# tuannv-github/srsRAN_Project

Measured on AMD Instinct MI355X. Metric: PDSCH+PUSCH codeblocks/s @ 100 MHz 273-PRB 4x4 MIMO (PDSCH 4 layers, PUSCH 4 layers x 4 rx), higher is better.
Workload: dtype int8+fp32; 1 GPU; BASELINE metric (PDSCH+PUSCH codeblocks/s @ 100 MHz 273-PRB 4x4 MIMO): full PDSCH+PUSCH slot pipeline, 100 MHz numerology-1 273 PRB, 256QAM R=948/1024; parallelism=single GPU

## Files before the change

srsran_project_amd/csrc/crc_api.cpp:

```cpp
#include "srsran_amd/crc.h"

#include <hip/hip_runtime.h>

#include "api_common.h"
#include "crc_args.h"
#include "crc_internal.h"
#include "ldpc_common.h"
#include <mutex>
#include <vector>

using namespace srs_amd;

struct srs_amd_crc_calculator {
  int         device   = 0;
  int         poly     = 0;
  uint32_t    polynom  = 0;
  int         order    = 0;
  uint32_t    max_bits = 0;
  uint32_t*   d_table  = nullptr;
  hipStream_t stream   = nullptr;
  void*       scratch  = nullptr;
  size_t      scratch_size = 0;
  uint32_t*   d_acc        = nullptr;
  uint32_t    acc_rows     = 0;
  std::mutex  mtx;
  ~srs_amd_crc_calculator()
  {
    (void)hipSetDevice(device);
    if (stream) {
      (void)hipStreamSynchronize(stream);
      (void)hipStreamDestroy(stream);
    }
    (void)hipFree(d_table);
    (void)hipFree(scratch);
    (void)hipFree(d_acc);
  }
};

namespace {

int check_rows(srs_amd_crc_calculator* crc, uint32_t stride, uint32_t nof_bits, uint32_t extra)
{
  if (crc == nullptr) {
    return fail(SRS_AMD_EINVAL, "null CRC calculator");
  }
  if (nof_bits > crc->max_bits) {
    return fail(SRS_AMD_EINVAL, "message of %u bits exceeds the calculator's %u", nof_bits, crc->max_bits);
  }
  if (static_cast<uint64_t>(stride) * 8 < static_cast<uint64_t>(nof_bits) + extra) {
    return fail(SRS_AMD_EINVAL, "row stride %u bytes too small for %u bits", stride, nof_bits + extra);
  }
  return SRS_AMD_OK;
}

int launch(srs_amd_crc_calculator* crc, uint32_t* d_out, uint8_t* d_bits, uint32_t stride, uint32_t nof_bits,
           uint32_t nof_rows, bool attach, hipStream_t stream)
{
  crc_args a{};
  a.bits      = d_bits;
  a.checksums = d_out;
  a.table     = crc->d_table;
  a.stride    = stride;
  a.nof_bits  = nof_bits;
  a.polynom   = crc->polynom;
  a.order     = static_cast<uint32_t>(crc->order);
  a.attach    = attach ? 1 : 0;
  hipError_t e = hipSetDevice(crc->device);
  if (e == hipSuccess && crc_needs_accumulator(nof_bits)) {
    if (crc->acc_rows < nof_rows) {
      (void)hipFree(crc->d_acc);
      crc->d_acc    = nullptr;
      crc->acc_rows = 0;
      e             = hipMalloc(&crc->d_acc, sizeof(uint32_t) * nof_rows);
      if (e == hipSuccess) {
        crc->acc_rows = nof_rows;
      }
    }
    a.acc = crc->d_acc;
  }
  if (e == hipSuccess) {
    e = launch_crc(a, nof_rows, stream);
  }
  return e == hipSuccess ? SRS_AMD_OK : hip_fail(e, "crc_kernel launch");
}

}

extern "C" {

int srs_amd_crc_calculator_create(srs_amd_crc_calculator** out, int poly, uint32_t max_bits, int device)
{
  if (out == nullptr) {
    return fail(SRS_AMD_EINVAL, "null handle pointer");
  }
  *out             = nullptr;
  uint32_t polynom = 0;
  int      order   = 0;
  if (!crc_params(poly, polynom, order)) {
    return fail(SRS_AMD_EINVAL, "Invalid CRC polynomial %d.", poly);
  }
  if (max_bits == 0 || max_bits > (1u << 26)) {
    return fail(SRS_AMD_EINVAL, "max_bits %u out of range", max_bits);
  }
  int rc = select_device(device);
  if (rc != SRS_AMD_OK) {
    return rc;
  }
  auto* c     = new srs_amd_crc_calculator();
  c->device   = device;
  c->poly     = poly;
  c->polynom  = polynom;
  c->order    = order;
  c->max_bits = max_bits;
  std::vector<uint32_t> t = crc_linear_table(poly, static_cast<int>(max_bits) + 32);
  hipError_t            e = hipMalloc(&c->d_table, t.size() * sizeof(uint32_t));
  if (e == hipSuccess) {
    e = hipMemcpy(c->d_table, t.data(), t.size() * sizeof(uint32_t), hipMemcpyHostToDevice);
  }
  if (e == hipSuccess) {
    e = hipStreamCreateWithFlags(&c->stream, hipStreamNonBlocking);
  }
  if (e != hipSuccess) {
    delete c;
    return hip_fail(e, "CRC table");
  }
  *out = c;
  return SRS_AMD_OK;
}

void srs_amd_crc_calculator_destroy(srs_amd_crc_calculator* crc)
{
  delete crc;
}

uint32_t srs_amd_crc_order(const srs_amd_crc_calculator* crc)
{
  return crc ? static_cast<uint32_t>(crc->order) : 0;
}

int srs_amd_crc_calculate_batch(srs_amd_crc_calculator* crc,
                                uint32_t*               d_checksums,
                                const uint8_t*          d_bits,
                                uint32_t                stride,
                                uint32_t                nof_bits,
                                uint32_t                nof_rows,
                                void*                   stream)
{
  int rc = check_rows(crc, stride, nof_bits, 0);
  if (rc != SRS_AMD_OK) {
    return rc;
  }
  if (nof_rows == 0) {
    return SRS_AMD_OK;
  }
  if (d_checksums == nullptr || (d_bits == nullptr && nof_bits > 0)) {
    return fail(SRS_AMD_EINVAL, "null device buffer");
  }
  std::lock_guard<std::mutex> lock(crc->mtx);
  return launch(crc, d_checksums, const_cast<uint8_t*>(d_bits), stride, nof_bits, nof_rows, false,
                static_cast<hipStream_t>(stream));
}

int srs_amd_crc_attach_batch(srs_amd_crc_calculator* crc,
                             uint8_t*                d_bits,
                             uint32_t                stride,
                             uint32_t                nof_bits,
                             uint32_t                nof_rows,
                             void*                   stream)
{
  int rc = check_rows(crc, stride, nof_bits, crc ? static_cast<uint32_t>(crc->order) : 0);
  if (rc != SRS_AMD_OK) {
// ... 10 lines not shown
}

int srs_amd_crc_calculate(srs_amd_crc_calculator* crc, uint32_t* checksum, const uint8_t* bits, uint32_t nof_bits)
{
  const uint32_t nbytes = (nof_bits + 7) / 8;
  int            rc     = check_rows(crc, nbytes, nof_bits, 0);
  if (rc != SRS_AMD_OK) {
    return rc;
  }
  if (checksum == nullptr || (bits == nullptr && nof_bits > 0)) {
    return fail(SRS_AMD_EINVAL, "null argument");
  }
  std::lock_guard<std::mutex> lock(crc->mtx);
  hipError_t                  e = hipSetDevice(crc->device);
  const size_t                need = 64 + nbytes;
  if (e == hipSuccess && need > crc->scratch_size) {
    (void)hipFree(crc->scratch);
    crc->scratch      = nullptr;
    crc->scratch_size = 0;
    e                 = hipMalloc(&crc->scratch, need);
    if (e == hipSuccess) {
      crc->scratch_size = need;
    }
  }
  if (e != hipSuccess) {
    return hip_fail(e, "CRC scratch");
  }
  auto* d_crc  = static_cast<uint32_t*>(crc->scratch);
  auto* d_bits = static_cast<uint8_t*>(crc->scratch) + 64;
  if (nbytes > 0) {
    e = hipMemcpyAsync(d_bits, bits, nbytes, hipMemcpyHostToDevice, crc->stream);
  }
  if (e != hipSuccess) {
    return hip_fail(e, "CRC upload");
  }
  rc = launch(crc, d_crc, d_bits, nbytes, nof_bits, 1, false, crc->stream);
  if (rc != SRS_AMD_OK) {
    return rc;
  }
  e = hipMemcpyAsync(checksum, d_crc, sizeof(uint32_t), hipMemcpyDeviceToHost, crc->stream);
  if (e == hipSuccess) {
    e = hipStreamSynchronize(crc->stream);
  }
  return e == hipSuccess ? SRS_AMD_OK : hip_fail(e, "CRC download");
}

}

const uint32_t* srs_amd::crc_device_table(const srs_amd_crc_calculator* crc)
{
  return crc ? crc->d_table : nullptr;
}

uint32_t srs_amd::crc_polynom(const srs_amd_crc_calculator* crc)
{
  return crc ? crc->polynom : 0;
}

uint32_t srs_amd::crc_order(const srs_amd_crc_calculator* crc)
{
  return crc ? static_cast<uint32_t>(crc->order) : 0;
}
```

srsran_project_amd/csrc/crc_device.h:

```cpp
#pragma once

#include <hip/hip_runtime.h>

#include <cstdint>

namespace srs_amd {

__device__ __forceinline__ uint32_t crc_wave_xor(uint32_t v)
{
#pragma unroll
  for (int o = 32; o >= 1; o >>= 1) {
    v ^= static_cast<uint32_t>(__shfl_xor(static_cast<int>(v), o, 64));
  }
  return v;
}

template <int THREADS>
__device__ __forceinline__ void crc_table8_init(uint32_t* T, uint32_t order, uint32_t polynom)
{
  if (order < 8) {
    return;
  }
  const uint32_t highbit = 1u << order;
  for (uint32_t t = threadIdx.x; t < 256; t += THREADS) {
// ... 73 lines not shown

__device__ __forceinline__ uint32_t crc_move(uint32_t R, uint32_t d, uint32_t order, const uint32_t* table)
{
  uint32_t out = 0;
#pragma unroll
  for (uint32_t j = 0; j < CRC_MAX_ORDER; ++j) {
    const uint32_t k    = j + d;
    const uint32_t word = k >= order ? table[k - order] : 0u;
    const uint32_t v    = k < order ? (1u << (k & 31u)) : word;
    out ^= (j < order) ? (v & (0u - ((R >> j) & 1u))) : 0u;
  }
  return out;
}

template <typename Fetch>
__device__ __forceinline__ uint32_t crc_chunk_rem(const Fetch& fetch, uint32_t b0, uint32_t b1, uint32_t order,
                                                  const uint32_t* T)
{
  const uint32_t mask = (1u << order) - 1u;
  const uint32_t sh   = order - 8;
  uint32_t       r    = 0;
  for (uint32_t b = b0; b < b1; b += CRC_FETCH_BATCH) {
    uint32_t v[CRC_FETCH_BATCH];
#pragma unroll
    for (uint32_t k = 0; k < CRC_FETCH_BATCH; ++k) {
      v[k] = b + k < b1 ? fetch(b + k) : 0u;
    }
#pragma unroll
    for (uint32_t k = 0; k < CRC_FETCH_BATCH; ++k) {
      if (b + k < b1) {
        r = T[r >> sh] ^ ((r << 8) & mask) ^ v[k];
      }
    }
  }
  return r;
}

__device__ __forceinline__ uint32_t crc_mulmod(uint32_t a, uint32_t c, uint32_t order, uint32_t polynom)
{
  const uint32_t mask = (1u << order) - 1u;
  const uint32_t top  = 1u << (order - 1);
  uint32_t       r    = 0;
#pragma unroll
  for (uint32_t i = 0; i < CRC_MAX_ORDER; ++i) {
    if (i < order) {
      r ^= c & (0u - ((a >> i) & 1u));
      const uint32_t hi = c & top;
      c                 = ((c << 1) & mask) ^ (hi ? (polynom & mask) : 0u);
    }
  }
  return r;
}

__device__ __forceinline__ uint32_t crc_xpow(uint32_t m, uint32_t order, const uint32_t* table)
{
  return m < order ? (1u << m) : table[m - order];
}

template <int THREADS>
__device__ __forceinline__ uint32_t crc_block_xor(uint32_t v, uint32_t* partial)
{
  v = crc_wave_xor(v);
  __syncthreads();
  if ((threadIdx.x & 63) == 0) {
    partial[threadIdx.x >> 6] = v;
  }
  __syncthreads();
  uint32_t crc = 0;
#pragma unroll
  for (int w = 0; w < THREADS / 64; ++w) {
    crc ^= partial[w];
  }
  return crc;
}

template <int THREADS, typename Fetch>
__device__ uint32_t block_crc_bytes(const Fetch&    fetch,
                                    uint32_t        n,
                                    uint32_t        order,
                                    uint32_t        polynom,
                                    const uint32_t* table,
                                    const uint32_t* T,
                                    uint32_t*       partial)
{
  const uint32_t nbytes = (n + 7) / 8;
  const uint32_t per    = (nbytes + THREADS - 1) / THREADS;
  const uint32_t b0     = threadIdx.x * per;
  const uint32_t b1     = min(nbytes, b0 + per);
  return crc_block_xor<THREADS>(crc_chunk_contrib(fetch, b0, b1, n, order, polynom, table, T), partial);
}

__device__ __forceinline__ void attach_crc_bits(uint8_t* row, uint32_t n, uint32_t order, uint32_t crc)
{
  const uint32_t first = n >> 3, last = (n + order - 1) >> 3;
  uint32_t       bytes[4];
#pragma unroll
  for (uint32_t k = 0; k < 4; ++k) {
    bytes[k] = first + k <= last ? row[first + k] : 0u;
  }
#pragma unroll
  for (uint32_t k = 0; k < 4; ++k) {
    if (first + k <= last) {
      uint32_t byte = bytes[k];
#pragma unroll
      for (uint32_t b = 0; b < 8; ++b) {
        const uint32_t pos = 8 * (first + k) + b;
// ... 49 lines not shown
```

srsran_project_amd/csrc/crc_internal.h:

```cpp
#pragma once

#include <cstdint>

#include "srsran_amd/crc.h"

namespace srs_amd {

const uint32_t* crc_device_table(const srs_amd_crc_calculator* crc);

uint32_t crc_polynom(const srs_amd_crc_calculator* crc);
uint32_t crc_order(const srs_amd_crc_calculator* crc);

}
```

srsran_project_amd/csrc/pusch_api.cpp:

```cpp
#include "srsran_amd/crc.h"
#include "srsran_amd/ldpc.h"
#include "srsran_amd/ldpc_rate_matching.h"
#include "srsran_amd/sch.h"

#include <hip/hip_runtime.h>

#include "api_common.h"
#include "crc_internal.h"
#include "device_buffer.h"
#include "ldpc_codec_internal.h"
#include "ldpc_common.h"
#include "rate_matching_common.h"
#include "pusch_processor_args.h"
#include "sch_args.h"
#include <cstring>
#include <algorithm>
#include <map>
#include <mutex>
#include <tuple>
#include <vector>

using namespace srs_amd;

struct srs_amd_pusch_decoder {
// ... 145 lines not shown
  if (internal && cfg->new_data && dematch_fused_enabled() && ldpc_hr_takes(static_cast<int>(p->base_graph),
                                                                             static_cast<int>(p->lifting_size), prefix)) {
    rm_geometry g{};
    const uint32_t e_max = std::max(p->rm_length_long, p->nof_short_segments > 0 ? p->rm_length_short : 0u);
    fuse = make_rm_geometry(g, p->base_graph, p->lifting_size, p->rv, p->modulation_order, p->Nref,
                            p->nof_filler_bits) == nullptr &&
           g.k0 == 0 && e_max <= g.L && e_max + g.F <= prefix;
    cw = ldpc_cw_rows{d_llrs, d->arrays.as<uint32_t>() + rows, d->arrays.as<uint32_t>(), p->modulation_order,
                      g.nof_info, g.F};
  }
  int rc = SRS_AMD_OK;
  if (!fuse) {
    rc = rate_dematch_batch_ex(d->dm, &md, cfg->new_data ? 1 : 0, d_llrs, d->arrays.as<uint32_t>() + rows,
                               d->arrays.as<uint32_t>(), d_soft, lay.row_bytes, rows, stream, internal,
                               internal ? prefix : 0);
  }
  if (rc != SRS_AMD_OK) {
    return rc;
  }
  const int crc_index = crc_index_of(p);
  const int crc_poly  = crc_poly_of(p);
  srs_amd_ldpc_decoder_config dc{};
  dc.base_graph      = p->base_graph;
  dc.lifting_size    = p->lifting_size;
  dc.nof_filler_bits = p->nof_filler_bits;
  dc.nof_crc_bits    = C > 1 ? p->nof_crc_bits : p->nof_tb_crc_bits;
  dc.max_iterations  = cfg->nof_ldpc_iterations;
  srs_amd_ldpc_decoder* dec = d->dec[cfg->force_decoding ? 1 : 0];
  const bool skip = !cfg->new_data && !internal;
  rc = ldpc_decode_batch_ex(dec, &dc, cfg->use_early_stop ? crc_poly : SRS_AMD_NO_CRC, d_soft, lay.row_bytes, nullptr,
                            prefix, d->msgs.as<uint8_t>(), msg_stride,
                            d->iters.as<int32_t>(), nullptr, rows, stream,
                            skip ? reinterpret_cast<const uint8_t*>(d_soft) + lay.flag_offset : nullptr, lay.row_bytes,
                            nullptr, fuse ? &cw : nullptr);
  if (rc != SRS_AMD_OK) {
    return rc;
  }
  if (!cfg->use_early_stop) {
    rc = srs_amd_crc_calculate_batch(d->crc[crc_index], d->checks.as<uint32_t>(), d->msgs.as<uint8_t>(), msg_stride,
                                     p->segment_length - p->nof_filler_bits, rows, stream);
    if (rc != SRS_AMD_OK) {
      return rc;
    }
  }
  assemble_args a{};
  a.msgs           = d->msgs.as<uint8_t>();
  a.iters          = d->iters.as<int32_t>();
  a.crc_checks     = cfg->use_early_stop ? nullptr : d->checks.as<uint32_t>();
  a.soft           = internal ? nullptr : reinterpret_cast<uint8_t*>(d_soft);
  a.tbs            = d_tbs;
  a.results        = d_results;
  a.cb_iterations  = d_cb_iterations;
  a.crc24a_table   = crc_device_table(d->crc[1]);
  a.acc            = d->tb_acc.as<uint32_t>();
  a.lay            = lay;
  a.msg_stride     = msg_stride;
  a.tb_stride      = tb_stride;
  a.nof_segments   = C;
  a.cb_info_bits   = p->cb_info_bits;
  a.tbs_bits       = p->tbs;
  a.max_iterations = cfg->nof_ldpc_iterations;
  a.new_data       = cfg->new_data ? 1 : 0;
  he               = launch_assemble(a, nof_tbs, stream);
  if (he == hipSuccess) {
    he = scope.close();
  }
  return he == hipSuccess ? SRS_AMD_OK : hip_fail(he, "assemble_kernel launch");
}

int decode_slot_locked(srs_amd_pusch_decoder*              d,
                       const srs_amd_pusch_decoder_config* cfg,
                       const srs_amd_pusch_ue*             ues,
                       uint32_t                            U,
                       const int8_t*                       d_llrs,
                       uint8_t*                            d_tbs,
                       srs_amd_pusch_decoder_result*       d_results,
                       const uint32_t*                     cb_offsets,
                       int32_t*                            d_cb_iterations,
                       hipStream_t                         stream,
                       const slot_harq*                    harq,
                       const slot_ue_patch*                patches,
                       uint32_t                            nof_patches)
{
  auto harq_of = [&](uint32_t u) -> const slot_harq* {
    return harq != nullptr && harq[u].soft != nullptr ? &harq[u] : nullptr;
  };
  struct bucket {
    uint32_t              bg, Z;
    int                   poly;
    bool                  mixed;
    uint32_t              prefix = 0, row0 = 0, rows = 0;
    std::vector<uint32_t> ues;
  };
  std::vector<bucket>                                          buckets;
  std::map<std::tuple<uint32_t, uint32_t, int, bool>, size_t> bucket_of;
  std::vector<uint32_t>                                        ue_prefix(U);
  uint32_t                                             S = 0, M = 0, R = 0, max_tb_bits = 0;
  for (uint32_t u = 0; u < U; ++u) {
    const srs_amd_sch_plan* p  = &ues[u].plan;
    int                     rc = check_plan(p);
    if (rc != SRS_AMD_OK) {
      return rc;
    }
    rm_geometry g{};
    if (const char* msg = make_rm_geometry(g, p->base_graph, p->lifting_size, p->rv, p->modulation_order, p->Nref,
                                           p->nof_filler_bits)) {
// ... 233 lines not shown
      rc = ldpc_decode_mixed(ldpc, b.bg, b.Z, cfg->nof_ldpc_iterations, soft + static_cast<size_t>(b.row0) * S, S,
                             reinterpret_cast<const uint32_t*>(dd + o_LEN) + b.row0,
                             d->msgs.as<uint8_t>() + static_cast<size_t>(b.row0) * M, M,
                             d->iters.as<int32_t>() + b.row0, b.rows, bs, d_F + b.row0,
                             dd + o_RD + sizeof(ldpc_row_desc) * b.row0);
      if (rc != SRS_AMD_OK) {
        return rc;
      }
      continue;
    }
    srs_amd_ldpc_decoder_config dc{};
    dc.base_graph     = b.bg;
    dc.lifting_size   = b.Z;
    dc.nof_crc_bits   = b.poly == 3 ? 16 : 24;
    dc.max_iterations = cfg->nof_ldpc_iterations;
    rc = ldpc_decode_batch_ex(ldpc, &dc, cfg->use_early_stop ? b.poly : SRS_AMD_NO_CRC,
                              soft + static_cast<size_t>(b.row0) * S, S, nullptr, b.prefix,
                              d->msgs.as<uint8_t>() + static_cast<size_t>(b.row0) * M, M,
                              d->iters.as<int32_t>() + b.row0, nullptr, b.rows, bs, nullptr, 0, d_F + b.row0);
    if (rc != SRS_AMD_OK) {
      return rc;
    }
  }
  he = d->fan.end(stream);
  if (he != hipSuccess) {
    return hip_fail(he, "PUSCH slot decoder stream join");
  }
  if (!cfg->use_early_stop) {
    for (uint32_t u = 0; u < U; ++u) {
      const srs_amd_sch_plan* p = &ues[u].plan;
      rc = srs_amd_crc_calculate_batch(d->crc[crc_index_of(p)], d->checks.as<uint32_t>() + tds[u].row0,
                                       d->msgs.as<uint8_t>() + static_cast<size_t>(tds[u].row0) * M, M,
                                       p->segment_length - p->nof_filler_bits, p->nof_segments, stream);
      if (rc != SRS_AMD_OK) {
        return rc;
      }
    }
  }
  if (ha.nof_rows != 0) {
    he = launch_harq_scatter(ha, max_soft, stream);
    if (he != hipSuccess) {
      return hip_fail(he, "harq_scatter_kernel launch");
    }
  }
  assemble_args a{};
  a.msgs           = d->msgs.as<uint8_t>();
  a.iters          = d->iters.as<int32_t>();
  a.crc_checks     = cfg->use_early_stop ? nullptr : d->checks.as<uint32_t>();
  a.soft           = nullptr;
  a.tbs            = d_tbs;
  a.results        = d_results;
  a.cb_iterations  = cb_offsets != nullptr ? d_cb_iterations : nullptr;
  a.crc24a_table   = crc_device_table(d->crc[1]);
  a.acc            = d->tb_acc.as<uint32_t>();
  a.msg_stride     = M;
  a.max_iterations = cfg->nof_ldpc_iterations;
  a.new_data       = 1;
  a.tds            = reinterpret_cast<const tb_desc*>(dd + o_TD);
  a.max_tb_bits    = max_tb_bits;
  he               = launch_assemble(a, U, stream);
  if (he == hipSuccess) {
    he = launch_harq_final(ha, stream);
  }
  if (he == hipSuccess) {
    he = scope.close();
  }
  return he == hipSuccess ? SRS_AMD_OK : hip_fail(he, "assemble_kernel launch");
}

int check_args(srs_amd_pusch_decoder* dec, const srs_amd_sch_plan* plan, const srs_amd_pusch_decoder_config* cfg)
{
  if (dec == nullptr || cfg == nullptr) {
    return fail(SRS_AMD_EINVAL, "null argument");
  }
  int rc = check_plan(plan);
  if (rc != SRS_AMD_OK) {
    return rc;
  }
  if (cfg->nof_ldpc_iterations == 0) {
    return fail(SRS_AMD_EINVAL, "The number of LDPC iterations must be positive.");
  }
  return SRS_AMD_OK;
}

}

extern "C" {

int srs_amd_pusch_decoder_create(srs_amd_pusch_decoder** out, int arith, int device)
{
  if (out == nullptr) {
    return fail(SRS_AMD_EINVAL, "null handle pointer");
  }
  *out = nullptr;
  if (arith != SRS_AMD_ARITH_SIMD && arith != SRS_AMD_ARITH_GENERIC) {
    return fail(SRS_AMD_EINVAL, "invalid LDPC arithmetic %d", arith);
  }
  int rc = select_device(device);
  if (rc != SRS_AMD_OK) {
    return rc;
  }
  auto* d   = new srs_amd_pusch_decoder();
  d->device = device;
  d->arith  = arith;
  rc        = srs_amd_crc_calculator_create(&d->crc[0], 3, 8448, device);
  if (rc == SRS_AMD_OK) {
// ... 224 lines not shown
```

srsran_project_amd/csrc/sch.hip:

```cpp
#include <hip/hip_runtime.h>

#include <cstdlib>

#include "crc_device.h"
#include "sch_args.h"

namespace srs_amd {
namespace {

constexpr int ASM_THREADS = 256;
constexpr uint32_t CRC24A_POLY = 0x1864cfb;
constexpr uint32_t SCH_MAX_SEGMENTS = 512;
constexpr uint32_t ASM_TB_PER       = 32;
constexpr uint32_t ASM_TB_CHUNK     = ASM_THREADS * ASM_TB_PER;

__device__ __forceinline__ uint32_t bit_at(const uint8_t* b, uint32_t p)
{
  return (b[p >> 3] >> (7 - (p & 7))) & 1u;
}

struct tb_gather {
  const uint8_t* base;
  uint32_t       stride;
  uint32_t       cbi;
  float          rcp;
  __device__ tb_gather(const uint8_t* base_, uint32_t stride_, uint32_t cbi_) :
    base(base_), stride(stride_), cbi(cbi_), rcp(1.0f / static_cast<float>(cbi_))
  {
  }
  __device__ uint32_t operator()(uint32_t j) const
  {
    uint32_t byte = 0;
    uint32_t b    = 8 * j;
    uint32_t r    = static_cast<uint32_t>(static_cast<float>(b) * rcp);
    int32_t  x    = static_cast<int32_t>(b - r * cbi);
    if (x < 0) {
      r -= 1;
      x += static_cast<int32_t>(cbi);
    } else if (x >= static_cast<int32_t>(cbi)) {
      r += 1;
      x -= static_cast<int32_t>(cbi);
    }
    uint32_t o = static_cast<uint32_t>(x);
    if (o + 8 <= cbi) {
      const uint8_t* m  = base + static_cast<size_t>(r) * stride + (o >> 3);
      const uint32_t sh = o & 7u;
      uint32_t       w  = static_cast<uint32_t>(m[0]) << 8;
      if (sh != 0) {
        w |= m[1];
      }
      return (w >> (8 - sh)) & 0xffu;
    }
    for (int k = 0; k < 8; ++k) {
      byte |= bit_at(base + static_cast<size_t>(r) * stride, o) << (7 - k);
      if (++o == cbi) {
        o = 0;
        ++r;
      }
    }
    return byte;
  }
};

__global__ __launch_bounds__(ASM_THREADS) void asm_copy_kernel(assemble_args a, uint32_t nof_cbs, uint32_t nw)
{
  const uint32_t x = blockIdx.x * ASM_THREADS + threadIdx.x;
  if (x >= nof_cbs * nw) {
    return;
  }
  const uint32_t cb   = x / nw;
  const uint32_t w    = x - cb * nw;
  uint8_t*       srow = a.soft + static_cast<size_t>(cb) * a.lay.row_bytes;
  if (!a.new_data && *reinterpret_cast<const int32_t*>(srow + a.lay.flag_offset) != 0) {
    return;
  }
  const uint32_t msg_bytes = a.lay.flag_offset - a.lay.msg_offset;
  const uint8_t* m         = a.msgs + static_cast<size_t>(cb) * a.msg_stride;
  if ((((reinterpret_cast<uintptr_t>(a.soft) | reinterpret_cast<uintptr_t>(a.msgs)) | a.lay.row_bytes |
        a.lay.msg_offset | a.msg_stride | msg_bytes) & 3u) == 0) {
    reinterpret_cast<uint32_t*>(srow + a.lay.msg_offset)[w] = reinterpret_cast<const uint32_t*>(m)[w];
    return;
  }
  for (uint32_t j = 4 * w; j < min(msg_bytes, 4 * w + 4); ++j) {
    srow[a.lay.msg_offset + j] = m[j];
  }
}

struct tb_view {
  uint8_t* tb;
  uint32_t row0, C, cbi, tbs_bits;
};

__device__ __forceinline__ tb_view view_of(const assemble_args& a, uint32_t t)
{
  if (a.tds != nullptr) {
    const tb_desc d = a.tds[t];
    return {a.tbs + d.tb_offset, d.row0, d.nof_segments, d.cb_info_bits, d.tbs_bits};
  }
  return {a.tbs + static_cast<size_t>(t) * a.tb_stride, t * a.nof_segments, a.nof_segments, a.cb_info_bits,
          a.tbs_bits};
}

__device__ __forceinline__ void assemble_tb(const assemble_args& a, uint32_t t, bool zero_acc)
{
  __shared__ uint32_t s_ok, s_sum, s_min, s_max, s_tb_ok;
  __shared__ uint8_t  s_fresh[SCH_MAX_SEGMENTS];
  __shared__ uint8_t  s_cb_ok[SCH_MAX_SEGMENTS];
  __shared__ uint16_t s_stat[SCH_MAX_SEGMENTS];
  const tb_view       v = view_of(a, t);
  if (zero_acc && threadIdx.x == 0 && a.acc != nullptr) {
    a.acc[t] = 0;
  }
  const uint32_t      C = v.C;
// ... 32 lines not shown
  __syncthreads();
  const uint8_t* src = a.msgs + static_cast<size_t>(v.row0) * a.msg_stride;
  if (a.soft) {
    for (uint32_t r = threadIdx.x; r < C; r += ASM_THREADS) {
      if (s_fresh[r]) {
        *reinterpret_cast<int32_t*>(a.soft + static_cast<size_t>(v.row0 + r) * a.lay.row_bytes + a.lay.flag_offset) =
            s_cb_ok[r] ? static_cast<int32_t>(s_stat[r]) : 0;
      }
    }
    __syncthreads();
    src = a.soft + static_cast<size_t>(v.row0) * a.lay.row_bytes + a.lay.msg_offset;
  }
  uint8_t*       tb     = v.tb;
  const uint32_t nbytes = v.tbs_bits / 8;
  const bool     all_ok = s_ok == C;
  if (C == 1) {
    if (all_ok) {
      for (uint32_t j = threadIdx.x; j < nbytes; j += ASM_THREADS) {
        tb[j] = src[j];
      }
    }
    if (threadIdx.x == 0) {
      s_tb_ok = all_ok ? 1 : 0;
    }
  }
  __syncthreads();
  if (threadIdx.x == 0) {
    srs_amd_pusch_decoder_result res{};
    res.tb_crc_ok             = static_cast<int32_t>(s_tb_ok);
    res.nof_codeblocks_total  = C;
    res.ldpc_iterations_sum   = s_sum;
    res.ldpc_iterations_min   = s_min;
    res.ldpc_iterations_max   = s_max;
    res.nof_codeblocks_crc_ok = s_ok;
    a.results[t]              = res;
  }
}

__global__ __launch_bounds__(ASM_THREADS) void assemble_kernel(assemble_args a)
{
  assemble_tb(a, blockIdx.x, true);
}

__device__ __forceinline__ const uint8_t* asm_source(const assemble_args& a, const tb_view& v, uint32_t& stride)
{
  if (a.soft) {
    stride = a.lay.row_bytes;
    return a.soft + static_cast<size_t>(v.row0) * a.lay.row_bytes + a.lay.msg_offset;
  }
  stride = a.msg_stride;
  return a.msgs + static_cast<size_t>(v.row0) * a.msg_stride;
}

struct lds_fetch {
  const uint8_t* chunk;
  uint32_t       first;
  __device__ uint32_t operator()(uint32_t j) const { return chunk[j - first]; }
};

__device__ __forceinline__ void asm_tb_chunk(const assemble_args& a, uint32_t t, uint32_t chunk, bool use_results)
{
  __shared__ uint32_t partial[ASM_THREADS / 64];
  __shared__ uint32_t T[256];
  __shared__ uint8_t  s_chunk[ASM_TB_CHUNK];
  __shared__ uint32_t s_bad;
  const tb_view       v = view_of(a, t);
  const uint32_t      c0 = chunk * ASM_TB_CHUNK;
  if (v.C == 1 || c0 >= v.tbs_bits / 8) {
    return;
  }
  if (use_results) {
    if (a.results[t].nof_codeblocks_crc_ok != v.C) {
      return;
    }
  } else {
    if (threadIdx.x == 0) {
      s_bad = 0;
    }
    __syncthreads();
    for (uint32_t r = threadIdx.x; r < v.C; r += ASM_THREADS) {
      const uint32_t cb = v.row0 + r;
      const bool     ok = a.crc_checks ? (a.crc_checks[cb] == 0) : (a.iters[cb] >= 0);
      if (!ok) {
        s_bad = 1;
      }
    }
    __syncthreads();
    if (s_bad != 0) {
      return;
    }
  }
  crc_table8_init<ASM_THREADS>(T, __builtin_amdgcn_readfirstlane(24u), __builtin_amdgcn_readfirstlane(CRC24A_POLY));
  uint32_t        stride;
  const uint8_t*  src    = asm_source(a, v, stride);
  const tb_gather g{src, stride, v.cbi};
  uint8_t*        tb     = v.tb;
  const uint32_t  nbytes = v.tbs_bits / 8;
  const uint32_t  n      = min(ASM_TB_CHUNK, nbytes - c0);
  constexpr uint32_t U = 8;
  for (uint32_t i0 = threadIdx.x; i0 < n; i0 += U * ASM_THREADS) {
    uint32_t v[U];
#pragma unroll
    for (uint32_t r = 0; r < U; ++r) {
      const uint32_t i = i0 + r * ASM_THREADS;
      v[r]             = i < n ? g(c0 + i) : 0u;
    }
#pragma unroll
    for (uint32_t r = 0; r < U; ++r) {
      const uint32_t i = i0 + r * ASM_THREADS;
      if (i < n) {
        s_chunk[i] = static_cast<uint8_t>(v[r]);
        tb[c0 + i] = static_cast<uint8_t>(v[r]);
      }
    }
  }
  __syncthreads();
  const uint32_t b0 = c0 + threadIdx.x * ASM_TB_PER;
  const uint32_t b1 = min(nbytes, b0 + ASM_TB_PER);
  const uint32_t to = min(v.tbs_bits, (c0 + ASM_TB_CHUNK) * 8);
  const uint32_t x  = crc_block_xor<ASM_THREADS>(
      crc_chunk_contrib(lds_fetch{s_chunk, c0}, b0, b1, v.tbs_bits, 24, CRC24A_POLY, a.crc24a_table, T, to),
      partial);
  if (threadIdx.x == 0 && x != 0) {
    atomicXor(a.acc + t, crc_move(x, v.tbs_bits - to, __builtin_amdgcn_readfirstlane(24u), a.crc24a_table));
  }
}

__global__ __launch_bounds__(ASM_THREADS) void asm_tb_kernel(assemble_args a)
{
  asm_tb_chunk(a, blockIdx.y, blockIdx.x, true);
}

__global__ __launch_bounds__(ASM_THREADS) void asm_merged_kernel(assemble_args a)
{
  if (blockIdx.x == gridDim.x - 1) {
    assemble_tb(a, blockIdx.y, false);
  } else {
    asm_tb_chunk(a, blockIdx.y, blockIdx.x, false);
  }
}

__global__ __launch_bounds__(64) void asm_final_kernel(assemble_args a, uint32_t nof_tbs)
{
  const uint32_t t = blockIdx.x * 64 + threadIdx.x;
  if (t >= nof_tbs) {
    return;
  }
  const tb_view  v = view_of(a, t);
  const uint32_t C = v.C;
  const uint32_t acc = a.acc != nullptr ? a.acc[t] : 0u;
  if (a.acc != nullptr) {
    a.acc[t] = 0;
  }
  if (C == 1 || a.results[t].nof_codeblocks_crc_ok != C) {
    return;
  }
  uint32_t       stride;
  const uint8_t* src = asm_source(a, v, stride);
  const uint32_t off = v.tbs_bits - (C - 1) * v.cbi;
  const uint8_t* m   = src + static_cast<size_t>(C - 1) * stride;
  uint32_t       chk = 0;
  for (uint32_t k = 0; k < 24; ++k) {
    chk = (chk << 1) | bit_at(m, off + k);
  }
  const bool ok           = acc == chk;
  a.results[t].tb_crc_ok  = ok ? 1 : 0;
  if (!ok && a.soft) {
    for (uint32_t r = 0; r < C; ++r) {
      uint8_t* srow = a.soft + static_cast<size_t>(v.row0 + r) * a.lay.row_bytes;
      *reinterpret_cast<int32_t*>(srow + a.lay.flag_offset) = 0;
    }
  }
}

}

constexpr uint32_t HARQ_THREADS = 256;
// ... 131 lines not shown
hipError_t launch_slot_row_patch(const slot_row_patch* items, uint32_t n, hipStream_t stream)
{
  if (n == 0) {
    return hipSuccess;
  }
  hipLaunchKernelGGL(slot_row_patch_kernel, dim3(n), dim3(64), 0, stream, items);
  return hipGetLastError();
}

hipError_t launch_harq_final(const harq_args& a, hipStream_t stream)
{
  if (a.nof_tbs == 0) {
    return hipSuccess;
  }
  hipLaunchKernelGGL(harq_final_kernel, dim3(a.nof_tbs), dim3(HARQ_THREADS), 0, stream, a);
  return hipGetLastError();
}


__global__ __launch_bounds__(256) void rm_arrays_kernel(uint32_t* arrays, uint32_t rows, uint32_t C, uint32_t S,
                                                       uint32_t e_short, uint32_t e_long, uint32_t tb_units)
{
  const uint32_t row = blockIdx.x * 256 + threadIdx.x;
  if (row < rows) {
    const uint32_t tb = row / C, r = row - tb * C;
    arrays[row]        = r < S ? e_short : e_long;
    arrays[rows + row] = tb * tb_units + (r < S ? r * e_short : S * e_short + (r - S) * e_long);
  }
}

hipError_t launch_rm_arrays(uint32_t* arrays, uint32_t nof_tbs, uint32_t C, uint32_t nof_short, uint32_t e_short,
                            uint32_t e_long, uint32_t tb_units, hipStream_t stream)
{
  const uint32_t rows = nof_tbs * C;
  hipLaunchKernelGGL(rm_arrays_kernel, dim3((rows + 255) / 256), dim3(256), 0, stream, arrays, rows, C, nof_short,
                     e_short, e_long, tb_units);
  return hipGetLastError();
}

hipError_t launch_assemble(const assemble_args& a, uint32_t nof_tbs, hipStream_t stream)
{
  if (nof_tbs == 0) {
    return hipSuccess;
  }
  if (a.soft) {
    const uint32_t nw  = (a.lay.flag_offset - a.lay.msg_offset + 3) / 4;
    const uint32_t ncb = nof_tbs * a.nof_segments;
    hipLaunchKernelGGL(asm_copy_kernel, dim3((ncb * nw + ASM_THREADS - 1) / ASM_THREADS), dim3(ASM_THREADS), 0,
                       stream, a, ncb, nw);
  }
  const uint32_t nbytes = (a.tds != nullptr ? a.max_tb_bits : a.tbs_bits) / 8;
  const char*    mv     = std::getenv("SRSRAN_AMD_ASM_MERGED");
  if (a.soft == nullptr && !(a.tds == nullptr && a.nof_segments == 1) && !(mv != nullptr && mv[0] == '0')) {
    hipLaunchKernelGGL(asm_merged_kernel, dim3((nbytes + ASM_TB_CHUNK - 1) / ASM_TB_CHUNK + 1, nof_tbs),
                       dim3(ASM_THREADS), 0, stream, a);
    hipError_t e = hipGetLastError();
    if (e != hipSuccess) {
      return e;
    }
    hipLaunchKernelGGL(asm_final_kernel, dim3((nof_tbs + 63) / 64), dim3(64), 0, stream, a, nof_tbs);
    return hipGetLastError();
  }
  hipLaunchKernelGGL(assemble_kernel, dim3(nof_tbs), dim3(ASM_THREADS), 0, stream, a);
  hipError_t e = hipGetLastError();
  if (e != hipSuccess || (a.tds == nullptr && a.nof_segments == 1)) {
    return e;
  }
  hipLaunchKernelGGL(asm_tb_kernel, dim3((nbytes + ASM_TB_CHUNK - 1) / ASM_TB_CHUNK, nof_tbs), dim3(ASM_THREADS), 0,
                     stream, a);
  e = hipGetLastError();
  if (e != hipSuccess) {
    return e;
  }
  hipLaunchKernelGGL(asm_final_kernel, dim3((nof_tbs + 63) / 64), dim3(64), 0, stream, a, nof_tbs);
  return hipGetLastError();
}

}
```

srsran_project_amd/csrc/sch_args.h:

```cpp
#pragma once

#include <hip/hip_runtime.h>

#include <cstdint>

#include "srsran_amd/sch.h"

namespace srs_amd {

struct rm_geometry;
struct enc_row_desc;

struct soft_row_layout {
  uint32_t soft_bytes;
  uint32_t msg_offset;
  uint32_t flag_offset;
  uint32_t row_bytes;
};

struct tb_desc {
  uint64_t tb_offset;
  uint32_t row0;
  uint32_t nof_segments;
  uint32_t cb_info_bits;
  uint32_t tbs_bits;
  uint32_t tb_crc_bits;
  uint32_t zero_pad;
  uint32_t msg_bytes;
  uint32_t pad;
};

struct pdsch_fused_args {
  const uint8_t*                 tbs;
  const tb_desc*                 tds;
  const uint32_t*                row_tb;
  const uint32_t*                row_E;
  const uint32_t*                row_out;
  const uint32_t*                row_geo;
  const struct rm_geometry*      geos;
  const struct enc_row_desc*     enc_rows;
  const uint32_t*                edges;
  uint32_t*                      tb_parts;
  uint32_t                       part_stride;
  const uint32_t*                crc16_table;
  const uint32_t*                crc24a_table;
  const uint32_t*                crc24b_table;
  uint32_t                       crc16_poly, crc24a_poly, crc24b_poly;
  uint8_t*                       cw;
  uint32_t                       nof_tbs;
  uint32_t                       nof_cbs;
  const uint32_t*                last_rows;
  uint32_t                       last_only;
  int32_t                        row_start[2][47];
};
hipError_t launch_pdsch_fused(const pdsch_fused_args& a, hipStream_t stream);

struct assemble_args {
  const uint8_t*                msgs;
  const int32_t*                iters;
  const uint32_t*               crc_checks;
  uint8_t*                      soft;
  uint8_t*                      tbs;
  srs_amd_pusch_decoder_result* results;
  int32_t*                      cb_iterations;
  const uint32_t*               crc24a_table;
  uint32_t*                     acc;
  soft_row_layout               lay;
  uint32_t                      msg_stride;
  uint32_t                      tb_stride;
  uint32_t                      nof_segments;
  uint32_t                      cb_info_bits;
  uint32_t                      tbs_bits;
  uint32_t                      max_iterations;
  int32_t                       new_data;
  const tb_desc*                tds;
  uint32_t                      max_tb_bits;
};

struct harq_row_desc {
  uint8_t* soft_row;
  uint32_t row;
  uint32_t soft_bytes;
  uint32_t msg_offset;
  uint32_t msg_bytes;
  uint32_t flag_offset;
  uint32_t new_data;
  uint32_t lazy;
  uint32_t tb_row0;
  uint32_t tb_C;
};
struct harq_tb_desc {
  uint8_t* soft;
  uint32_t result;
  uint32_t C;
  uint32_t row_bytes;
  uint32_t flag_offset;
  uint32_t lazy;
  uint32_t row0;
  uint32_t soft_bytes;
};
struct harq_args {
  const harq_row_desc*          rows;
  uint32_t                      nof_rows;
  const harq_tb_desc*           tbs;
  uint32_t                      nof_tbs;
  int8_t*                       internal;
  uint32_t                      S;
  uint8_t*                      msgs;
  uint32_t                      M;
  int32_t*                      iters;
  int32_t*                      prev;
  srs_amd_pusch_decoder_result* results;
};
hipError_t launch_harq_gather(const harq_args& a, uint32_t max_soft_bytes, hipStream_t stream);
hipError_t launch_harq_scatter(const harq_args& a, uint32_t max_soft_bytes, hipStream_t stream);
hipError_t launch_harq_final(const harq_args& a, hipStream_t stream);

struct slot_row_patch {
// ... 16 lines not shown
```

Before: 24.77 million codeblocks/s.

## Use slice-by-4 CRC24A tables with 16-byte word gathers in TB assembly

Replaces the per-byte LDS staging and bytewise table-driven CRC in the PUSCH transport-block assembly with a 16-byte-per-thread scheme. Each thread gathers 16 aligned bytes with word loads and alignbyte, writes them with a single 16-byte store, and folds them using precomputed slice-by-4 tables plus a power-of-x table to shift each partial CRC. The host precomputes and uploads these tables at CRC creation, which removes the in-kernel table build. This adds unaligned-edge handling and more complex boundary logic, and halves bytes per thread from 32 to 16, which changes the grid size.

```diff
diff --git a/srsran_project_amd/csrc/crc_api.cpp b/srsran_project_amd/csrc/crc_api.cpp
--- a/srsran_project_amd/csrc/crc_api.cpp
+++ b/srsran_project_amd/csrc/crc_api.cpp
@@ -4,8 +4,10 @@
 
 #include "api_common.h"
 #include "crc_args.h"
+#include "crc_device.h"
 #include "crc_internal.h"
 #include "ldpc_common.h"
+#include <algorithm>
 #include <mutex>
 #include <vector>
 
@@ -18,6 +20,7 @@
   int         order    = 0;
   uint32_t    max_bits = 0;
   uint32_t*   d_table  = nullptr;
+  uint32_t*   d_slices = nullptr;
   hipStream_t stream   = nullptr;
   void*       scratch  = nullptr;
   size_t      scratch_size = 0;
@@ -32,6 +35,7 @@
       (void)hipStreamDestroy(stream);
     }
     (void)hipFree(d_table);
+    (void)hipFree(d_slices);
     (void)hipFree(scratch);
     (void)hipFree(d_acc);
   }
@@ -51,6 +55,35 @@
     return fail(SRS_AMD_EINVAL, "row stride %u bytes too small for %u bits", stride, nof_bits + extra);
   }
   return SRS_AMD_OK;
+}
+
+std::vector<uint32_t> slice_tables(uint32_t polynom, int order)
+{
+  const uint32_t        highbit = 1u << order;
+  const uint32_t        top     = 8 * CRC_SLICE_PIECE * 255 + 1;
+  std::vector<uint32_t> xp(std::max<uint32_t>(top, order + 32));
+  uint32_t              r = 1;
+  for (uint32_t m = 0; m < xp.size(); ++m) {
+    xp[m] = r;
+    r <<= 1;
+    if (r & highbit) {
+      r ^= polynom;
+    }
+  }
+  std::vector<uint32_t> t(CRC_SLICE_WORDS, 0);
+  for (uint32_t m = 0; m < 4; ++m) {
+    for (uint32_t v = 0; v < 256; ++v) {
+      uint32_t x = 0;
+      for (uint32_t i = 0; i < 8; ++i) {
+        x ^= ((v >> i) & 1u) ? xp[order + 8 * m + i] : 0u;
+      }
+      t[256 * m + v] = x;
+    }
+  }
+  for (uint32_t k = 0; k < 256; ++k) {
+    t[1024 + k] = xp[8 * CRC_SLICE_PIECE * k];
+  }
+  return t;
 }
 
 int launch(srs_amd_crc_calculator* crc, uint32_t* d_out, uint8_t* d_bits, uint32_t stride, uint32_t nof_bits,
@@ -117,6 +150,13 @@
   if (e == hipSuccess) {
     e = hipMemcpy(c->d_table, t.data(), t.size() * sizeof(uint32_t), hipMemcpyHostToDevice);
   }
+  if (e == hipSuccess && order >= 8) {
+    const std::vector<uint32_t> sl = slice_tables(polynom, order);
+    e                              = hipMalloc(&c->d_slices, sl.size() * sizeof(uint32_t));
+    if (e == hipSuccess) {
+      e = hipMemcpy(c->d_slices, sl.data(), sl.size() * sizeof(uint32_t), hipMemcpyHostToDevice);
+    }
+  }
   if (e == hipSuccess) {
     e = hipStreamCreateWithFlags(&c->stream, hipStreamNonBlocking);
   }
@@ -233,6 +273,11 @@
   return crc ? crc->d_table : nullptr;
 }
 
+const uint32_t* srs_amd::crc_device_slices(const srs_amd_crc_calculator* crc)
+{
+  return crc ? crc->d_slices : nullptr;
+}
+
 uint32_t srs_amd::crc_polynom(const srs_amd_crc_calculator* crc)
 {
   return crc ? crc->polynom : 0;
diff --git a/srsran_project_amd/csrc/crc_device.h b/srsran_project_amd/csrc/crc_device.h
--- a/srsran_project_amd/csrc/crc_device.h
+++ b/srsran_project_amd/csrc/crc_device.h
@@ -149,6 +149,25 @@
   return r;
 }
 
+constexpr uint32_t CRC_SLICE_PIECE = 16;
+constexpr uint32_t CRC_SLICE_WORDS = 5 * 256;
+
+__device__ __forceinline__ uint32_t crc24_fold4(uint32_t r, uint32_t w, const uint32_t* S)
+{
+  return (w & 0xffffffu) ^ S[w >> 24] ^ S[256 + (r & 0xffu)] ^ S[512 + ((r >> 8) & 0xffu)] ^ S[768 + (r >> 16)];
+}
+
+__device__ __forceinline__ uint32_t crc24_fold16(const uint32_t p[4], const uint32_t* S)
+{
+  const uint32_t w0 = __builtin_bswap32(p[0]);
+  uint32_t       r  = (w0 & 0xffffffu) ^ S[w0 >> 24];
+#pragma unroll
+  for (int i = 1; i < 4; ++i) {
+    r = crc24_fold4(r, __builtin_bswap32(p[i]), S);
+  }
+  return r;
+}
+
 __device__ __forceinline__ uint32_t crc_xpow(uint32_t m, uint32_t order, const uint32_t* table)
 {
   return m < order ? (1u << m) : table[m - order];
diff --git a/srsran_project_amd/csrc/crc_internal.h b/srsran_project_amd/csrc/crc_internal.h
--- a/srsran_project_amd/csrc/crc_internal.h
+++ b/srsran_project_amd/csrc/crc_internal.h
@@ -8,6 +8,8 @@
 
 const uint32_t* crc_device_table(const srs_amd_crc_calculator* crc);
 
+const uint32_t* crc_device_slices(const srs_amd_crc_calculator* crc);
+
 uint32_t crc_polynom(const srs_amd_crc_calculator* crc);
 uint32_t crc_order(const srs_amd_crc_calculator* crc);
 
diff --git a/srsran_project_amd/csrc/pusch_api.cpp b/srsran_project_amd/csrc/pusch_api.cpp
--- a/srsran_project_amd/csrc/pusch_api.cpp
+++ b/srsran_project_amd/csrc/pusch_api.cpp
@@ -221,6 +221,7 @@
   a.results        = d_results;
   a.cb_iterations  = d_cb_iterations;
   a.crc24a_table   = crc_device_table(d->crc[1]);
+  a.crc24a_slices  = crc_device_slices(d->crc[1]);
   a.acc            = d->tb_acc.as<uint32_t>();
   a.lay            = lay;
   a.msg_stride     = msg_stride;
@@ -560,6 +561,7 @@
   a.results        = d_results;
   a.cb_iterations  = cb_offsets != nullptr ? d_cb_iterations : nullptr;
   a.crc24a_table   = crc_device_table(d->crc[1]);
+  a.crc24a_slices  = crc_device_slices(d->crc[1]);
   a.acc            = d->tb_acc.as<uint32_t>();
   a.msg_stride     = M;
   a.max_iterations = cfg->nof_ldpc_iterations;
diff --git a/srsran_project_amd/csrc/sch.hip b/srsran_project_amd/csrc/sch.hip
--- a/srsran_project_amd/csrc/sch.hip
+++ b/srsran_project_amd/csrc/sch.hip
@@ -11,8 +11,14 @@
 constexpr int ASM_THREADS = 256;
 constexpr uint32_t CRC24A_POLY = 0x1864cfb;
 constexpr uint32_t SCH_MAX_SEGMENTS = 512;
-constexpr uint32_t ASM_TB_PER       = 32;
+constexpr uint32_t ASM_TB_PER       = CRC_SLICE_PIECE;
 constexpr uint32_t ASM_TB_CHUNK     = ASM_THREADS * ASM_TB_PER;
+static_assert(ASM_TB_PER == 16 && ASM_THREADS == 256, "piece16, the 16-byte store and the 256-entry piece table");
+
+constexpr uint32_t asm_tb_chunks(uint32_t nbytes)
+{
+  return (nbytes + 15 + ASM_TB_CHUNK - 1) / ASM_TB_CHUNK;
+}
 
 __device__ __forceinline__ uint32_t bit_at(const uint8_t* b, uint32_t p)
 {
@@ -28,12 +34,10 @@
     base(base_), stride(stride_), cbi(cbi_), rcp(1.0f / static_cast<float>(cbi_))
   {
   }
-  __device__ uint32_t operator()(uint32_t j) const
+  __device__ void locate(uint32_t b, uint32_t& r, uint32_t& o) const
   {
-    uint32_t byte = 0;
-    uint32_t b    = 8 * j;
-    uint32_t r    = static_cast<uint32_t>(static_cast<float>(b) * rcp);
-    int32_t  x    = static_cast<int32_t>(b - r * cbi);
+    r         = static_cast<uint32_t>(static_cast<float>(b) * rcp);
+    int32_t x = static_cast<int32_t>(b - r * cbi);
     if (x < 0) {
       r -= 1;
       x += static_cast<int32_t>(cbi);
@@ -41,7 +45,13 @@
       r += 1;
       x -= static_cast<int32_t>(cbi);
     }
-    uint32_t o = static_cast<uint32_t>(x);
+    o = static_cast<uint32_t>(x);
+  }
+  __device__ uint32_t operator()(uint32_t j) const
+  {
+    uint32_t byte = 0;
+    uint32_t r, o;
+    locate(8 * j, r, o);
     if (o + 8 <= cbi) {
       const uint8_t* m  = base + static_cast<size_t>(r) * stride + (o >> 3);
       const uint32_t sh = o & 7u;
@@ -59,6 +69,35 @@
       }
     }
     return byte;
+  }
+  __device__ bool words_ok() const
+  {
+    return (cbi & 7u) == 0 && cbi >= 128 && ((reinterpret_cast<uintptr_t>(base) | stride) & 3u) == 0;
+  }
+  __device__ void piece16(uint32_t j0, uint32_t out[4]) const
+  {
+    uint32_t r, o;
+    locate(8 * j0, r, o);
+    o >>= 3;
+    const uint32_t  n1   = min(16u, (cbi >> 3) - o);
+    const uintptr_t row2 = reinterpret_cast<uintptr_t>(base) + static_cast<size_t>(r + 1) * stride;
+    const uintptr_t p1   = row2 - stride + o;
+    const uintptr_t q2   = row2 - n1;
+    const uint32_t  sh1 = static_cast<uint32_t>(p1 & 3u), sh2 = static_cast<uint32_t>(q2 & 3u);
+    const uintptr_t a1 = p1 & ~uintptr_t(3), a2 = q2 & ~uintptr_t(3);
+    uint32_t        w1[5], w2[5];
+#pragma unroll
+    for (uint32_t i = 0; i < 5; ++i) {
+      w1[i] = 4 * i < sh1 + n1 ? reinterpret_cast<const uint32_t*>(a1)[i] : 0u;
+      w2[i] = n1 < 16 && a2 + 4 * i >= row2 && a2 + 4 * i < q2 + 16 ? reinterpret_cast<const uint32_t*>(a2)[i] : 0u;
+    }
+#pragma unroll
+    for (uint32_t i = 0; i < 4; ++i) {
+      const uint32_t x = __builtin_amdgcn_alignbyte(w1[i + 1], w1[i], sh1);
+      const uint32_t y = __builtin_amdgcn_alignbyte(w2[i + 1], w2[i], sh2);
+      const uint32_t m = n1 >= 4 * i + 4 ? 0xffffffffu : n1 <= 4 * i ? 0u : (1u << (8 * (n1 - 4 * i))) - 1u;
+      out[i]           = (x & m) | (y & ~m);
+    }
   }
 };
 
@@ -197,21 +236,17 @@
   return a.msgs + static_cast<size_t>(v.row0) * a.msg_stride;
 }
 
-struct lds_fetch {
-  const uint8_t* chunk;
-  uint32_t       first;
-  __device__ uint32_t operator()(uint32_t j) const { return chunk[j - first]; }
-};
-
 __device__ __forceinline__ void asm_tb_chunk(const assemble_args& a, uint32_t t, uint32_t chunk, bool use_results)
 {
   __shared__ uint32_t partial[ASM_THREADS / 64];
-  __shared__ uint32_t T[256];
-  __shared__ uint8_t  s_chunk[ASM_TB_CHUNK];
+  __shared__ uint32_t S[1024];
   __shared__ uint32_t s_bad;
-  const tb_view       v = view_of(a, t);
-  const uint32_t      c0 = chunk * ASM_TB_CHUNK;
-  if (v.C == 1 || c0 >= v.tbs_bits / 8) {
+  const tb_view       v      = view_of(a, t);
+  const uint32_t      nbytes = v.tbs_bits / 8;
+  const uint32_t      lead   = static_cast<uint32_t>(reinterpret_cast<uintptr_t>(v.tb) & 15u);
+  const uint32_t      end    = lead + nbytes;
+  const uint32_t      c0     = chunk * ASM_TB_CHUNK;
+  if (v.C == 1 || c0 >= end) {
     return;
   }
   if (use_results) {
@@ -235,39 +270,55 @@
       return;
     }
   }
-  crc_table8_init<ASM_THREADS>(T, __builtin_amdgcn_readfirstlane(24u), __builtin_amdgcn_readfirstlane(CRC24A_POLY));
+  for (uint32_t k = threadIdx.x; k < 1024; k += ASM_THREADS) {
+    S[k] = a.crc24a_slices[k];
+  }
   uint32_t        stride;
-  const uint8_t*  src    = asm_source(a, v, stride);
+  const uint8_t*  src = asm_source(a, v, stride);
   const tb_gather g{src, stride, v.cbi};
-  uint8_t*        tb     = v.tb;
-  const uint32_t  nbytes = v.tbs_bits / 8;
-  const uint32_t  n      = min(ASM_TB_CHUNK, nbytes - c0);
-  constexpr uint32_t U = 8;
-  for (uint32_t i0 = threadIdx.x; i0 < n; i0 += U * ASM_THREADS) {
-    uint32_t v[U];
+  uint8_t*        tb  = v.tb;
+  const uint32_t  u0  = c0 + threadIdx.x * ASM_TB_PER;
+  const uint32_t ref    = min(c0 + ASM_TB_CHUNK, end & ~15u);
+  const bool     whole  = u0 + ASM_TB_PER <= ref;
+  const bool     inside = whole && u0 >= lead;
+  const uint32_t xpow   = whole ? a.crc24a_slices[1024 + (ref - u0) / ASM_TB_PER - 1] : 0u;
+  uint32_t       p[4]   = {0u, 0u, 0u, 0u};
+  if (inside && g.words_ok()) {
+    g.piece16(u0 - lead, p);
+  } else if (u0 < end) {
 #pragma unroll
-    for (uint32_t r = 0; r < U; ++r) {
-      const uint32_t i = i0 + r * ASM_THREADS;
-      v[r]             = i < n ? g(c0 + i) : 0u;
-    }
+    for (uint32_t k = 0; k < ASM_TB_PER; ++k) {
+      const uint32_t u = u0 + k;
+      if (u >= lead && u < end) {
+        const uint32_t byte = g(u - lead);
+        p[k / 4] |= byte << (8 * (k % 4));
+        if (!inside) {
+          tb[u - lead] = static_cast<uint8_t>(byte);
+        }
+      }
+    }
+  }
+  if (inside) {
+    *reinterpret_cast<uint4*>(tb + (u0 - lead)) = make_uint4(p[0], p[1], p[2], p[3]);
+  }
+  __syncthreads();
+  const uint32_t x = crc_block_xor<ASM_THREADS>(
+      whole ? crc_mulmod(crc24_fold16(p, S), xpow, 24, CRC24A_POLY) : 0u, partial);
+  if (threadIdx.x == 0 && x != 0) {
+    atomicXor(a.acc + t, crc_move(x, 8 * (end - ref) + 24, __builtin_amdgcn_readfirstlane(24u), a.crc24a_table));
+  }
+  if (!whole && u0 < end) {
+    uint32_t r = 0;
 #pragma unroll
-    for (uint32_t r = 0; r < U; ++r) {
-      const uint32_t i = i0 + r * ASM_THREADS;
-      if (i < n) {
-        s_chunk[i] = static_cast<uint8_t>(v[r]);
-        tb[c0 + i] = static_cast<uint8_t>(v[r]);
-      }
-    }
-  }
-  __syncthreads();
-  const uint32_t b0 = c0 + threadIdx.x * ASM_TB_PER;
-  const uint32_t b1 = min(nbytes, b0 + ASM_TB_PER);
-  const uint32_t to = min(v.tbs_bits, (c0 + ASM_TB_CHUNK) * 8);
-  const uint32_t x  = crc_block_xor<ASM_THREADS>(
-      crc_chunk_contrib(lds_fetch{s_chunk, c0}, b0, b1, v.tbs_bits, 24, CRC24A_POLY, a.crc24a_table, T, to),
-      partial);
-  if (threadIdx.x == 0 && x != 0) {
-    atomicXor(a.acc + t, crc_move(x, v.tbs_bits - to, __builtin_amdgcn_readfirstlane(24u), a.crc24a_table));
+    for (uint32_t k = 0; k < ASM_TB_PER + 3; ++k) {
+      if (k < end - u0 + 3) {
+        const uint32_t byte = k < ASM_TB_PER ? (p[(k % ASM_TB_PER) / 4] >> (8 * (k % 4))) & 0xffu : 0u;
+        r                   = S[r >> 16] ^ ((r << 8) & 0xffffffu) ^ (k < end - u0 ? byte : 0u);
+      }
+    }
+    if (r != 0) {
+      atomicXor(a.acc + t, r);
+    }
   }
 }
 
@@ -505,7 +556,7 @@
   const uint32_t nbytes = (a.tds != nullptr ? a.max_tb_bits : a.tbs_bits) / 8;
   const char*    mv     = std::getenv("SRSRAN_AMD_ASM_MERGED");
   if (a.soft == nullptr && !(a.tds == nullptr && a.nof_segments == 1) && !(mv != nullptr && mv[0] == '0')) {
-    hipLaunchKernelGGL(asm_merged_kernel, dim3((nbytes + ASM_TB_CHUNK - 1) / ASM_TB_CHUNK + 1, nof_tbs),
+    hipLaunchKernelGGL(asm_merged_kernel, dim3(asm_tb_chunks(nbytes) + 1, nof_tbs),
                        dim3(ASM_THREADS), 0, stream, a);
     hipError_t e = hipGetLastError();
     if (e != hipSuccess) {
@@ -519,8 +570,7 @@
   if (e != hipSuccess || (a.tds == nullptr && a.nof_segments == 1)) {
     return e;
   }
-  hipLaunchKernelGGL(asm_tb_kernel, dim3((nbytes + ASM_TB_CHUNK - 1) / ASM_TB_CHUNK, nof_tbs), dim3(ASM_THREADS), 0,
-                     stream, a);
+  hipLaunchKernelGGL(asm_tb_kernel, dim3(asm_tb_chunks(nbytes), nof_tbs), dim3(ASM_THREADS), 0, stream, a);
   e = hipGetLastError();
   if (e != hipSuccess) {
     return e;
diff --git a/srsran_project_amd/csrc/sch_args.h b/srsran_project_amd/csrc/sch_args.h
--- a/srsran_project_amd/csrc/sch_args.h
+++ b/srsran_project_amd/csrc/sch_args.h
@@ -64,6 +64,7 @@
   srs_amd_pusch_decoder_result* results;
   int32_t*                      cb_iterations;
   const uint32_t*               crc24a_table;
+  const uint32_t*               crc24a_slices;
   uint32_t*                     acc;
   soft_row_layout               lay;
   uint32_t                      msg_stride;
```

Result: no change. 24.83 million codeblocks/s (median of 5 runs) (+0.2%).
